# bitsauce/Carla-ppo

Measured on AMD Instinct MI355X. Metric: VAE+PPO train frames/sec on 160×80×3 synthetic obs at 1/2/4/8 MI355X, higher is better.
Workload: dtype bf16; 1 GPU; ConvVAE SGD step (fwd+ELBO+bwd+TF-Adam), batch=512 per GPU, 160x80x3 frames, z_dim=64, rgb target (BASELINE configs[1]; global batch 512); global_batch=512, parallelism=single, frames_resident_in_hbm=2048, frame_table=uint8 camera bytes, k/255 in registers, noise=N(0,1) drawn inside the reparameterisation kernel (Philox4x32-10), launch=eager launches: one C call per step (mi_vae_train_step), storage=bf16 activations/weights, fp32 accumulate, fp32 master weights+Adam

## Files before the change

### carla-ppo_amd/csrc/conv_ops.hip

```cpp
#include <stdlib.h>
#include "gemm_core.hpp"
#include "tallk_tile.hpp"
#include "mi_internal.hpp"
#include "mi355_carla.h"

using namespace mi;

namespace {

inline int esz_of(int dtype) { return dtype == MI_BF16 ? 2 : 4; }
inline bool dtype_ok(int dtype) { return dtype == MI_F32 || dtype == MI_BF16 || dtype == MI_BF16X3; }

template <typename T, typename TIn, int AMODE, int BMODE, int VA, int AALIGN>
int launch_gemm_bn(hipStream_t st, const GemmParams& p, int M_for_grid, int gz) {
    const int gx = (M_for_grid + GEMM_BM - 1) / GEMM_BM;
    if (gx <= 0) return MI_OK;
    if (p.N <= 32) {
        dim3 g(gx, 1, gz);
        MI_LAUNCH((gemm_kernel<T, TIn, AMODE, BMODE, VA, AALIGN, 32>), g, dim3(GEMM_NT), 0, st, p);
    } else if (p.N <= 64) {
        dim3 g(gx, 1, gz);
        MI_LAUNCH((gemm_kernel<T, TIn, AMODE, BMODE, VA, AALIGN, 64>), g, dim3(GEMM_NT), 0, st, p);
    } else {
        dim3 g(gx, (p.N + 127) / 128, gz);
// ... 835 lines not shown
}
extern "C" int mi_small_reduce_flush(void* stream) {
    if (t_sr.njobs == 0) return MI_OK;
    if ((hipStream_t)stream != t_sr_stream) {
        const int rc = sr_launch_params(t_sr_stream, t_sr);
        return rc != MI_OK ? rc : mi_fail(MI_ERR_STATE, "mi_small_reduce_flush: the recorded jobs belong to another stream (issued there)");
    }
    return sr_launch_params(t_sr_stream, t_sr);
}
extern "C" int mi_small_reduce_deferring(void) { return t_sr_defer; }

bool mi_narrow_enabled() { return narrow_enabled(); }

void mi_get_trace(long long** buf, int* cap) { *buf = g_trace; *cap = g_trace_cap; }

static bool tallk_enabled() {
    static int on = -1;
    if (on < 0) { const char* e = getenv("MI355_TALLK"); on = (e && e[0] == '0') ? 0 : 1; }
    return on != 0;
}

extern "C" {

int mi_debug_set_trace(void* dev_ptr, int capacity_entries) { g_trace = (long long*)dev_ptr; g_trace_cap = dev_ptr ? capacity_entries : 0; return MI_OK; }

int mi_set_tuning(int key, int value) {
    int prev;
    if (key == 0) { prev = gemm2_enabled() ? 1 : 0; g_gemm2_on = value ? 1 : 0; }
    else if (key == 1) { prev = tapconv_minblocks(); g_tap_min = value < 0 ? -1 : value; }
    else if (key == 2) { prev = g_wgrad_skip; g_wgrad_skip = value; }
    else if (key == 5) { prev = g_tap_variant; g_tap_variant = value; }
    else if (key == 6) { prev = g_tap_direct; g_tap_direct = value ? 1 : 0; }
    else if (key == 8) { prev = 0; }
    else if (key == 4) { prev = narrow_enabled() ? 1 : 0; g_narrow_on = value ? 1 : 0; }
    else if (key == 3) { prev = tapwgrad_enabled() ? 1 : 0; g_tapwgrad_on = value ? 1 : 0; }
    else if (key == 7) { prev = g_tapwgrad_split; g_tapwgrad_split = value ? 1 : 0; }
    else if (key == 9) { prev = g_tapwgrad_blocks; g_tapwgrad_blocks = value < 16 ? 16 : value; }
    else if (key == 10) { prev = g_nw_waves; g_nw_waves = value; }
    else if (key == 12) { prev = g_tap_mask_prefetch; g_tap_mask_prefetch = value ? 1 : 0; }
    else if (key == 11) { prev = g_dense_wgrad_blocks; g_dense_wgrad_blocks = value < 1 ? 1 : value; }
    else if (key == 13) { prev = mi_rwconv_mode(value < 0 ? 0 : value); }
    else if (key == 14) { prev = g_tapwgrad_cw; g_tapwgrad_cw = value ? 1 : 0; }
    else if (key == 15) { prev = mi_rwconv_conv_mode(value < 0 ? 0 : value); }
    else if (key == 16) { prev = mi_rwconv_blocks(value < 0 ? 0 : value); }
    else if (key == 17) { prev = g_gemm2_tile; g_gemm2_tile = value; }
    else if (key == 18) { prev = g_slab_bf16; g_slab_bf16 = value ? 1 : 0; }
    else if (key == 19) { prev = g_nw_depth; g_nw_depth = value; }
    else if (key == 20) { prev = g_gemm2_stages; g_gemm2_stages = value; }
    else if (key == 21) { prev = g_x3_tapwgrad; g_x3_tapwgrad = value; }
    else if (key == 22) { prev = g_dwgs_on; g_dwgs_on = value ? 1 : 0; }
    else if (key == 24) { prev = g_tw_ldec; g_tw_ldec = value < 0 || value > 3 ? 0 : value; }
    else if (key == 25) { prev = g_dectail_dbg; g_dectail_dbg = value; }
    else if (key == 26) { prev = g_dectail_split5; g_dectail_split5 = value ? 1 : 0; }
    else if (key == 23) { prev = mi_enc12_debug(value); }
    else return mi_fail(MI_ERR_ARG, "mi_set_tuning: unknown key");
    return prev;
}

int mi_conv2d_nhwc_fwd(void* stream, int dtype, const void* x, const int* frame_idx, int x_is_f32,
                       int B, int IH, int IW, int Cin, const void* w, int w_transposed, const float* bias, int KH, int KW, int Cout,
                       int relu, void* out) {
    return mi_conv2d_nhwc_fwd_bits(stream, dtype, x, frame_idx, x_is_f32, B, IH, IW, Cin, w, w_transposed, bias, KH, KW, Cout, relu, out, nullptr, nullptr);
}

int mi_conv2d_nhwc_fwd_bits(void* stream, int dtype, const void* x, const int* frame_idx, int x_is_f32,
                            int B, int IH, int IW, int Cin, const void* w, int w_transposed, const float* bias, int KH, int KW, int Cout,
                            int relu, void* out, void* relu_bits, int* wrote_bits) {
    const void* const wfrag = mi_rwconv_take_wfrag();
    const int OH = (IH - KH) / 2 + 1, OW = (IW - KW) / 2 + 1;
    if (wrote_bits) *wrote_bits = 0;
    if (w_transposed) {
        const int r4 = try_narrow_conv((hipStream_t)stream, dtype, x, x_is_f32 == 2 ? 2 : ((x_is_f32 || dtype == MI_F32) ? 1 : (dtype == MI_BF16X3 ? 3 : 0)), frame_idx, w, B, IH, IW, Cin, KH, KW, Cout, bias, relu, nullptr, out,
                                       (dtype == MI_BF16 && relu && Cout == 32) ? relu_bits : nullptr);
        if (r4 > 0 && wrote_bits && relu_bits && dtype == MI_BF16 && relu && Cout == 32) *wrote_bits = 1;
        if (r4 != 0) return r4 > 0 ? MI_OK : r4;
    }
    if (x_is_f32 == 2) return mi_fail(MI_ERR_ARG, "mi_conv2d_nhwc_fwd: uint8 frames are only read by the narrow-layer kernel (bf16 mode, 1..3 channels -> 32, K-contiguous weights)");
    GemmParams p = {};
    p.a = x; p.a_frame_idx = frame_idx;
    fill_conv_geom(p, B, IH, IW, Cin, OH, OW, KH, KW, 2, needs_merge(Cin, dtype, x_is_f32));
    p.N = Cout; p.b = w; p.ldb = w_transposed ? p.K : Cout; p.b_vec = vec_ok(w, p.ldb, dtype);
    p.out = out; p.bias = bias; p.mask = nullptr; p.relu = relu; p.out_f32 = 0; p.ksplit_len = 0;
    if (w_transposed) return conv_form_gemm<B_NK>((hipStream_t)stream, dtype, x_is_f32, p, 1, wfrag);
    return conv_form_gemm<B_KN>((hipStream_t)stream, dtype, x_is_f32, p, 1);
}

int mi_conv2d_nhwc_dgrad(void* stream, int dtype, const void* dy, int B, int OH, int OW, int Cout,
                         const void* w, int KH, int KW, int Cin, int IH, int IW, const void* mask, void* dx) {
    return mi_conv2d_nhwc_dgrad_bits(stream, dtype, dy, B, OH, OW, Cout, w, KH, KW, Cin, IH, IW, mask, nullptr, dx);
}

int mi_conv2d_nhwc_dgrad_bits(void* stream, int dtype, const void* dy, int B, int OH, int OW, int Cout,
                              const void* w, int KH, int KW, int Cin, int IH, int IW, const void* mask, const void* mask_bits, void* dx) {
    if (mask_bits) {
        const int r5 = mi_try_rwconv_gather((hipStream_t)stream, dtype, dy, w, B, OH, OW, Cout, IH, IW, Cin, KH, KW, dx, nullptr, mask, 0, mask_bits, nullptr, nullptr);
        if (r5 != 0) return r5 > 0 ? MI_OK : r5;
    }
    GemmParams p = {};
    p.a = dy; p.b = w; p.ldb = 0; p.b_vec = 1;
    p.out = dx; p.bias = nullptr; p.mask = mask; p.relu = 0; p.out_f32 = 0;
    return deconv_form_gemm((hipStream_t)stream, dtype, p, B, OH, OW, Cout, IH, IW, Cin, KH, KW);
}

int mi_conv2d_nhwc_wgrad(void* stream, int dtype, const void* x, const int* frame_idx, int x_is_f32,
                         int B, int IH, int IW, int Cin, const void* dy, int KH, int KW, int Cout, float* dw) {
    return mi_conv2d_nhwc_wgrad_ws(stream, dtype, x, frame_idx, x_is_f32, B, IH, IW, Cin, dy, KH, KW, Cout, dw, nullptr, 0, nullptr);
// ... 327 lines not shown
```

### carla-ppo_amd/csrc/enc12.hip

```cpp
#include <stdlib.h>
#include "enc12_tile.hpp"
#include "mi_internal.hpp"
#include "mi355_carla.h"

using namespace mi;

static int g_enc12_dbg = 0;
int mi_enc12_debug(int mask) { const int prev = g_enc12_dbg; g_enc12_dbg = mask < 0 ? 0 : mask; return prev; }

static int enc12_grid(int u8) {
    static int resident[2];
    if (!resident[u8]) {
        int per_cu = 0, dev = 0, cus = 256;
        hipDeviceProp_t pr;
        const void* fn = u8 ? (const void*)enc12_fwd_kernel<unsigned char> : (const void*)enc12_fwd_kernel<float>;
        if (hipOccupancyMaxActiveBlocksPerMultiprocessor(&per_cu, fn, 256, 0) != hipSuccess || per_cu < 1) per_cu = 2;
        if (hipGetDevice(&dev) == hipSuccess && hipGetDeviceProperties(&pr, dev) == hipSuccess) cus = pr.multiProcessorCount;
        resident[u8] = per_cu * cus;
    }
    return resident[u8];
}

extern "C" int mi_conv2d_enc12_fwd(void* stream, int dtype, const void* frames, int frames_fmt, const int* frame_idx, int B, int FH, int FW, const void* w1_t, const float* b1,
                                   const void* w2_t, const float* b2, void* act1, void* relu_bits1, void* act2, int* launched) {
    const void* const w2f = mi_rwconv_take_wfrag();
    if (!launched || !frames || !w1_t || !b1 || !w2_t || !b2 || !act1 || !act2) return mi_fail(MI_ERR_ARG, "mi_conv2d_enc12_fwd: missing buffers");
    *launched = 0;
    static int on = -1;
    if (on < 0) { const char* e = getenv("MI355_ENC12"); on = (e && e[0] == '0') ? 0 : 1; }
    if (!on || !mi_narrow_enabled() || dtype != MI_BF16 || (frames_fmt != 1 && frames_fmt != 2) || B < 1 || FH != 80 || FW != 160) return MI_OK;
    if ((((uintptr_t)frames) & (frames_fmt == 2 ? 1 : 7)) || (((uintptr_t)w1_t) | ((uintptr_t)w2_t) | ((uintptr_t)b1) | ((uintptr_t)b2) | ((uintptr_t)act1) | ((uintptr_t)act2)) & 15) return MI_OK;
    if (relu_bits1 && (((uintptr_t)relu_bits1) & 3)) return MI_OK;
    if ((long long)B * 3 >= (1ll << 30)) return MI_OK;
    Enc12Params q = {};
    q.frames = frames; q.frame_idx = frame_idx; q.frame_stride = (long long)FH * FW * 3;
    q.w1 = (const bf16_t*)w1_t; q.b1 = b1; q.w2 = (const bf16_t*)w2_t; q.b2 = b2;
    q.act1 = (bf16_t*)act1; q.bits1 = (uint32_t*)relu_bits1; q.act2 = (bf16_t*)act2;
    q.w2f = (const bf16_t*)w2f;
    q.B = B; q.ntiles = 3 * B;
    int nblocks = enc12_grid(frames_fmt == 2 ? 1 : 0);
    if (nblocks > q.ntiles) nblocks = q.ntiles;
    static int ring = -1;
    if (ring < 0) { const char* e = getenv("MI355_ENC12_RING"); ring = (e && e[0] == '0') ? 0 : 1; }
    static int c2 = -1;
    if (c2 < 0) { const char* e = getenv("MI355_ENC12_C2"); c2 = (e && e[0] == '0') ? 0 : 1; }
    int use_ring = ring, use_c2 = c2;
    int dbg = g_enc12_dbg;
    if (dbg & 4096) { use_ring = (dbg >> 13) & 1; use_c2 = (dbg >> 14) & 1; dbg = 0; }
    if (dbg && frames_fmt == 2) {
        q.dbg = dbg;
        if (dbg & 2048) MI_LAUNCH((enc12_fwd_kernel<unsigned char, 1, 1, 1>), dim3(nblocks), dim3(256), 0, (hipStream_t)stream, q);
        else MI_LAUNCH((enc12_fwd_kernel<unsigned char, 1>), dim3(nblocks), dim3(256), 0, (hipStream_t)stream, q);
    } else if (use_ring && use_c2 && frames_fmt == 2) MI_LAUNCH((enc12_fwd_kernel<unsigned char, 0, 1, 1>), dim3(nblocks), dim3(256), 0, (hipStream_t)stream, q);
    else if (use_ring && frames_fmt == 2) MI_LAUNCH((enc12_fwd_kernel<unsigned char, 0, 1>), dim3(nblocks), dim3(256), 0, (hipStream_t)stream, q);
    else if (frames_fmt == 2) MI_LAUNCH(enc12_fwd_kernel<unsigned char>, dim3(nblocks), dim3(256), 0, (hipStream_t)stream, q);
    else MI_LAUNCH(enc12_fwd_kernel<float>, dim3(nblocks), dim3(256), 0, (hipStream_t)stream, q);
    const int rc = mi_check_launch("enc12_fwd_kernel");
    if (rc == MI_OK) *launched = 1;
    return rc;
}
```

### carla-ppo_amd/csrc/enc12_tile.hpp

```cpp
#pragma once
#include "wgrad_tile.hpp"

namespace mi {

typedef uint32_t e12_u32x4 __attribute__((ext_vector_type(4)));

constexpr int E12_PW = 40;
constexpr int E12_ROWS = 15;
constexpr int E12_PLANE = E12_ROWS * E12_PW * 64;
constexpr int E12_LDS = 2 * E12_PLANE;

struct Enc12Params {
    const void* frames; const int* frame_idx; long long frame_stride;
    const bf16_t* w1; const float* b1;
    const bf16_t* w2; const float* b2;
    const bf16_t* w2f;
    bf16_t* act1; uint32_t* bits1;
    bf16_t* act2;
    int B, ntiles;
    int dbg;
};

template <int IMM> __device__ __forceinline__ void e12_lds_read(u16x8& d, uint32_t addr) { asm volatile("ds_read_b128 %0, %1 offset:%2" : "=&v"(d) : "v"(addr), "n"(IMM)); }
template <int N> __device__ __forceinline__ void e12_lds_wait(u16x8& d) { asm volatile("s_waitcnt lgkmcnt(%1)" : "+v"(d) : "n"(N)); }
template <int F> __device__ __forceinline__ void e12_frag_read(u16x8& d, const uint32_t (&base)[2][2]) {
    constexpr int kh = F >> 3, kw = (F >> 1) & 3, ks = F & 1;
    e12_lds_read<(kw & 1) * E12_PLANE + kh * E12_PW * 64>(d, base[kw >> 1][ks]);
}
template <int F, int NF> struct E12Conv2Pipe {
    static __device__ __forceinline__ void run(u16x8 (&fb)[NF], const u16x8 (&wf2)[32], f32x16& acc, const uint32_t (&base)[2][2]) {
        constexpr int issued = F == 0 ? NF - 1 : (F - 2 + NF < 31 ? F - 2 + NF : 31);
        e12_lds_wait<issued - F>(fb[F % NF]);
        acc = __builtin_amdgcn_mfma_f32_32x32x16_bf16(__builtin_bit_cast(bf16x8, wf2[F]), __builtin_bit_cast(bf16x8, fb[F % NF]), acc, 0, 0, 0);
        if constexpr (F >= 1 && F - 1 + NF < 32) e12_frag_read<F - 1 + NF>(fb[(F - 1) % NF], base);
        if constexpr (F + 1 < 32) E12Conv2Pipe<F + 1, NF>::run(fb, wf2, acc, base);
    }
};
template <int F, int NF> struct E12Conv2Prologue {
    static __device__ __forceinline__ void run(u16x8 (&fb)[NF], const uint32_t (&base)[2][2]) {
        e12_frag_read<F>(fb[F], base);
        if constexpr (F + 1 < NF) E12Conv2Prologue<F + 1, NF>::run(fb, base);
    }
};

template <typename TS, int DBG = 0, int RING = 0, int C2 = 0>
__global__ __launch_bounds__(256) __attribute__((amdgpu_waves_per_eu(2, 2))) void enc12_fwd_kernel(const Enc12Params p) {
    const int dbg = DBG ? p.dbg : 0;
    constexpr int SSZ = (int)sizeof(TS), GSZ = 4 * SSZ, GDW = GSZ / 4;
    constexpr int FW = 160, A1H = 39, A1W = 79, A2H = 18, A2W = 38;
    __shared__ __attribute__((aligned(1024))) unsigned char lds[E12_LDS];
    const int tid = threadIdx.x, lane = tid & 63;
    const int wave = __builtin_amdgcn_readfirstlane(tid >> 6);
    const int lrow = lane & 31, lgrp = lane >> 5;

    const int nt = wave & 1, mh = wave >> 1;
    u16x8 wf1[3], wf2[32];
    {
        const __amdgpu_buffer_rsrc_t rsW1 = __builtin_amdgcn_make_buffer_rsrc((void*)p.w1, 0, 32 * 48 * 2, 0x00020000);
        const bool w2frag = p.w2f != nullptr;
        const __amdgpu_buffer_rsrc_t rsW2 = __builtin_amdgcn_make_buffer_rsrc((void*)(w2frag ? p.w2f : p.w2), 0, 64 * 512 * 2, 0x00020000);
#pragma unroll
        for (int s = 0; s < 3; ++s) wf1[s] = __builtin_bit_cast(u16x8, __builtin_amdgcn_raw_buffer_load_b128(rsW1, (lrow * 48 + s * 16 + lgrp * 8) * 2, 0, 0));
#pragma unroll
        for (int f = 0; f < 32; ++f)
            wf2[f] = __builtin_bit_cast(u16x8, __builtin_amdgcn_raw_buffer_load_b128(rsW2, w2frag ? ((nt * 32 + f) * 64 + lane) * 16 : ((nt * 32 + lrow) * 512 + f * 16 + lgrp * 8) * 2, 0, 0));
    }
    f32x16 acc1_0, acc2_0;
#pragma unroll
    for (int qd = 0; qd < 4; ++qd) {
        const f32x4 ba = *(const f32x4*)(p.b1 + 8 * qd + 4 * lgrp), bb = *(const f32x4*)(p.b2 + nt * 32 + 8 * qd + 4 * lgrp);
#pragma unroll
        for (int t = 0; t < 4; ++t) { acc1_0[4 * qd + t] = ba[t]; acc2_0[4 * qd + t] = bb[t]; }
    }
    const uint32_t rowb = (uint32_t)(FW * 3 * SSZ);
    uint32_t goff[6];
#pragma unroll
    for (int j = 0; j < 6; ++j) {
        const int qa = 4 * (j >> 1) + (j & 1), qb = qa + 2;
        goff[j] = lgrp ? (uint32_t)(qb / 3) * rowb + (uint32_t)((qb % 3) * GSZ) : (uint32_t)(qa / 3) * rowb + (uint32_t)((qa % 3) * GSZ);
    }
    struct Raw { uint32_t d[6][GDW]; };

    const int G = (int)gridDim.x;
    struct Band { int b, band, y0, npix, own_rows, ngrp; const unsigned char* fbase; };
    auto band_of = [&](int tile) -> Band {
        Band q;
        q.b = tile / 3; q.band = tile - 3 * q.b; q.y0 = 12 * q.band;
        const int nrows = q.band == 2 ? 15 : 14;
        q.npix = nrows * A1W; q.own_rows = q.band == 2 ? 15 : 12;
        q.ngrp = (q.npix + 31) >> 5;
        long long fr = q.b;
        if constexpr (RING && SSZ == 1) {
            if (p.frame_idx) {
                int v;
                asm volatile("s_load_dword %0, %1, 0x0\n\ts_waitcnt lgkmcnt(0)" : "=s"(v) : "s"(p.frame_idx + q.b));
                fr = v;
            }
        } else if (p.frame_idx) fr = p.frame_idx[q.b];
        q.fbase = (const unsigned char*)p.frames + fr * p.frame_stride * SSZ;
        return q;
    };
    auto request3 = [&](const unsigned char* fbase, int y0r, int npixr, int grp, Raw& r) {
        const int pq = min(grp * 32 + lrow, npixr - 1);
        const int row = pq / A1W, col = pq - row * A1W;
        const unsigned char* pix = fbase + (2 * (y0r + row) * FW + 2 * col) * 3 * SSZ;
        if constexpr (RING && SSZ == 1) {
#pragma unroll
            for (int j = 0; j < 6; ++j) {
                if (dbg & 16) { r.d[j][0] = 0x40404040u + (uint32_t)pq; continue; }
                asm volatile("global_load_dword %0, %1, off" : "=&v"(r.d[j][0]) : "v"(pix + goff[j]));
            }
            return;
        }
#pragma unroll
        for (int j = 0; j < 6; ++j) {
            if (dbg & 16) {
#pragma unroll
                for (int e = 0; e < GDW; ++e) r.d[j][e] = 0x40404040u + (uint32_t)pq;
                continue;
            }
            const PackU<uint32_t, GDW, 2> v = *(const PackU<uint32_t, GDW, 2>*)(pix + goff[j]);
#pragma unroll
            for (int e = 0; e < GDW; ++e) r.d[j][e] = v.v[e];
        }
    };
    auto request = [&](const Band& q, int grp, Raw& r) { request3(q.fbase, q.y0, q.npix, grp, r); };
    auto ring_wait = [&](Raw& r) {
        if constexpr (RING && SSZ == 1)
            asm volatile("s_waitcnt vmcnt(%6)" : "+v"(r.d[0][0]), "+v"(r.d[1][0]), "+v"(r.d[2][0]), "+v"(r.d[3][0]), "+v"(r.d[4][0]), "+v"(r.d[5][0]) : "n"(6 * ((SSZ == 1 ? 3 : 2) - 1)));
    };
    constexpr bool DEEP = SSZ == 1;
    constexpr int NB = DEEP ? 3 : 2;
    Raw r0, r1, ra, rb, rc;
    int tile = (int)blockIdx.x;
    if (tile >= p.ntiles) return;
    Band cb = band_of(tile);
    if constexpr (RING) {
        request(cb, wave, ra); request(cb, wave + 4, rb);
        if constexpr (NB == 3) request(cb, wave + 8, rc);
    } else {
        request(cb, min(wave, cb.ngrp - 1), r0);
        if constexpr (DEEP) request(cb, min(wave + 4, cb.ngrp - 1), r1);
    }
    for (; tile < p.ntiles; tile += G) {
        const int b = cb.b, band = cb.band, y0 = cb.y0, npix = cb.npix, own_rows = cb.own_rows, ngrp = cb.ngrp;

        if constexpr (RING) {
            const int nsteps = (ngrp - wave + 3) >> 2, nsp = (nsteps + NB - 1) / NB * NB;
            const bool more = tile + G < p.ntiles;
            const Band nb = more ? band_of(tile + G) : cb;
            auto step = [&](Raw& cur, int k) {
                const int grp = wave + 4 * k;
                ring_wait(cur);
                u16x8 xf[3];
    #pragma unroll
                for (int j = 0; j < 6; ++j) {
                    uint32_t* dst = (uint32_t*)&xf[j >> 1] + 2 * (j & 1);
                    float f[4];
                    if constexpr (SSZ == 1) {
    #pragma unroll
                        for (int e = 0; e < 4; ++e) f[e] = (float)((cur.d[j][0] >> (8 * e)) & 255u) * U8_RCP255;
                    } else {
    #pragma unroll
                        for (int e = 0; e < 4; ++e) f[e] = __builtin_bit_cast(float, cur.d[j][e < GDW ? e : 0]);
// ... 188 lines not shown
```

### carla-ppo_amd/csrc/enchead.hip

```cpp
#include <stdlib.h>
#include "enchead_tile.hpp"
#include "mi_internal.hpp"
#include "mi355_carla.h"

using namespace mi;

namespace mi {
__global__ __launch_bounds__(1024) void enchead_reduce_kernel(const float* __restrict__ slabs, int n, float* __restrict__ dw, float* __restrict__ db) {
    __shared__ float red[32][33];
    const int c = threadIdx.x & 31, r0 = threadIdx.x >> 5;
    const bool bias = blockIdx.x == 48;
    const int col = bias ? 64 * 32 + c : (int)blockIdx.x * 32 + c;
    float s = 0.f;
    for (int k0 = r0; k0 < n; k0 += 256) {
        float v[8];
#pragma unroll
        for (int u = 0; u < 8; ++u) { const int k = k0 + 32 * u; v[u] = k < n ? __builtin_nontemporal_load(&slabs[(long long)k * EH_SLAB + col]) : 0.f; }
#pragma unroll
        for (int u = 0; u < 8; ++u) s += v[u];
    }
    red[r0][c] = s;
    __syncthreads();
    if (threadIdx.x < 32) {
        float t = 0.f;
#pragma unroll
        for (int r = 0; r < 32; ++r) t += red[r][threadIdx.x];
        if (bias) db[threadIdx.x] += t; else dw[col] += t;
    }
}
}

static int enchead_grid(int u8) {
    static int resident[2];
    if (!resident[u8]) {
        int per_cu = 0, dev = 0, cus = 256;
        hipDeviceProp_t pr;
        const void* fn = u8 ? (const void*)enchead_bwd_kernel<unsigned char> : (const void*)enchead_bwd_kernel<float>;
        if (hipOccupancyMaxActiveBlocksPerMultiprocessor(&per_cu, fn, 256, 0) != hipSuccess || per_cu < 1) per_cu = 2;
        if (hipGetDevice(&dev) == hipSuccess && hipGetDeviceProperties(&pr, dev) == hipSuccess) cus = pr.multiProcessorCount;
        resident[u8] = per_cu * cus;
    }
    return resident[u8];
}

extern "C" int mi_conv2d_head_bwd_blocks(void) { const int a = enchead_grid(0), b = enchead_grid(1); return a > b ? a : b; }

extern "C" int mi_conv2d_head_bwd_fused(void* stream, int dtype, const void* frames, int frames_fmt, const int* frame_idx, int B, int FH, int FW,
                                        const void* dy2, const void* w2, const void* bits_act1, float* dw1, float* db1, void* scratch, long long scratch_bytes, int* n_blocks) {
    if (!n_blocks || !frames || !dy2 || !w2 || !dw1 || !db1) return mi_fail(MI_ERR_ARG, "mi_conv2d_head_bwd_fused: missing buffers");
    *n_blocks = 0;
    static int on = -1;
    if (on < 0) { const char* e = getenv("MI355_ENCHEAD"); on = (e && e[0] == '0') ? 0 : 1; }
    if (!on || !mi_narrow_enabled() || dtype != MI_BF16 || !bits_act1 || !scratch || B < 1) return MI_OK;
    if (frames_fmt != 1 && frames_fmt != 2) return MI_OK;
    if (FH < 10 || FW < 10) return MI_OK;
    const int IH = (FH - 4) / 2 + 1, IW = (FW - 4) / 2 + 1;
    if (IH < 4 || IW < 4) return MI_OK;
    const int OH = (IH - 4) / 2 + 1, OW = (IW - 4) / 2 + 1;
    const int ssz = frames_fmt == 2 ? 1 : 4;
    if ((((uintptr_t)frames) & (2 * ssz - 1)) || ((long long)FW * 3 * ssz) % (2 * ssz) != 0 || ((long long)FH * FW * 3 * ssz) % (2 * ssz) != 0) return MI_OK;
    if ((((uintptr_t)dy2) | ((uintptr_t)w2) | ((uintptr_t)scratch) | ((uintptr_t)dw1) | ((uintptr_t)db1)) & 15) return MI_OK;
    if ((long long)B * OH * OW * 128 >= 0x7fffff00ll || (long long)B * IH * IW * 8 >= 0x7fffff00ll) return MI_OK;
    EncHeadParams q = {};
    q.dy = (const bf16_t*)dy2; q.dy_bytes = (unsigned)((long long)B * OH * OW * 128); q.B = B; q.OH = OH; q.OW = OW;
    q.w = (const bf16_t*)w2; q.bits = (const uint32_t*)bits_act1; q.bits_bytes = (unsigned)((long long)B * IH * IW * 8);
    q.frames = frames; q.frame_idx = frame_idx; q.frame_stride = (long long)FH * FW * 3;
    q.IH = IH; q.IW = IW; q.FW = FW;
    const int tiles_y = (IH + EH_TY - 1) / EH_TY;
    q.tiles_x = (IW + EH_TX - 1) / EH_TX; q.tiles_per_frame = tiles_y * q.tiles_x;
    const long long ntiles = (long long)B * q.tiles_per_frame;
    if (ntiles >= (1ll << 30)) return MI_OK;
    q.ntiles = (int)ntiles; q.div_tpf = make_fastdiv(q.tiles_per_frame); q.div_tx = make_fastdiv(q.tiles_x);
    int nblocks = enchead_grid(frames_fmt == 2 ? 1 : 0);
    if (nblocks > q.ntiles) nblocks = q.ntiles;
    if (nblocks >= 16) nblocks &= ~7;
    if (scratch_bytes < (long long)nblocks * EH_SLAB * 4) return MI_OK;
    q.slabs = (float*)scratch;
    hipStream_t st = (hipStream_t)stream;
    if (frames_fmt == 2) MI_LAUNCH(enchead_bwd_kernel<unsigned char>, dim3(nblocks), dim3(256), 0, st, q);
    else MI_LAUNCH(enchead_bwd_kernel<float>, dim3(nblocks), dim3(256), 0, st, q);
    int rc = mi_check_launch("enchead_bwd_kernel");
    if (rc != MI_OK) return rc;
    if (mi_small_reduce_deferring()) {
        rc = mi_reduce_slabs(st, q.slabs, (long long)EH_SLAB, nblocks, 48ll * 32, dw1);
        if (rc == MI_OK) rc = mi_reduce_slabs(st, q.slabs + 64 * 32, (long long)EH_SLAB, nblocks, 32ll, db1);
    } else {
        MI_LAUNCH(enchead_reduce_kernel, dim3(49), dim3(1024), 0, st, (const float*)q.slabs, nblocks, dw1, db1);
        rc = mi_check_launch("enchead_reduce_kernel");
    }
    if (rc == MI_OK) *n_blocks = nblocks;
    return rc;
}
```

### carla-ppo_amd/csrc/enchead_tile.hpp

```cpp
#pragma once
#include "wgrad_tile.hpp"

namespace mi {

constexpr int EH_TY = 8, EH_TX = 16;
constexpr int EH_SR = EH_TY / 2 + 1, EH_SC = EH_TX / 2 + 1;
constexpr int EH_NS = EH_SR * EH_SC;
constexpr int EH_SP = 144;
constexpr int EH_DYS = (EH_NS * EH_SP + 255) & ~255;
constexpr int EH_GP = 80;
constexpr int EH_GT = 32 * EH_GP;
constexpr int EH_SLAB = 64 * 32 + 32;
constexpr int EH_PT = 32 * 128;

struct EncHeadParams {
    const bf16_t* dy; unsigned dy_bytes; int B, OH, OW;
    const bf16_t* w;
    const uint32_t* bits; unsigned bits_bytes;
    const void* frames; const int* frame_idx; long long frame_stride;
    int IH, IW, FW;
    float* slabs;
    int tiles_x, tiles_per_frame, ntiles;
    FastDiv div_tpf, div_tx;
};

template <typename TS>
__global__ __launch_bounds__(256) __attribute__((amdgpu_waves_per_eu(3, 4))) void enchead_bwd_kernel(const EncHeadParams p) {
    constexpr int SSZ = (int)sizeof(TS), GSZ = 4 * SSZ, GDW = GSZ / 4;
    __shared__ __attribute__((aligned(1024))) unsigned char lds[EH_DYS + 4 * EH_PT + 4 * EH_GT + 4 * 4096];
    unsigned char* const dys = lds;
    const int tid = threadIdx.x, lane = tid & 63;
    const int wave = __builtin_amdgcn_readfirstlane(tid >> 6);
    const int lrow = lane & 31, lgrp = lane >> 5;
    unsigned char* const ptw = lds + EH_DYS + wave * EH_PT;
    unsigned char* const gtw = lds + EH_DYS + 4 * EH_PT + wave * EH_GT;
    const int ph = wave >> 1, pw = wave & 1;
    const int li = lrow >> 3, lj = lrow & 7;
    typedef __attribute__((address_space(3))) s16x4* lds_v4;

    unsigned char* const wlw = lds + EH_DYS + 4 * EH_PT + 4 * EH_GT + wave * 4096;
    u16x8 wf[3][4];
    {
        const __amdgpu_buffer_rsrc_t rsW = __builtin_amdgcn_make_buffer_rsrc((void*)p.w, 0, 16 * 32 * 64 * 2, 0x00020000);
#pragma unroll
        for (int tap = 0; tap < 4; ++tap) {
            const int kh = ph + 2 * (tap >> 1), kw = pw + 2 * (tap & 1);
#pragma unroll
            for (int kk = 0; kk < 4; ++kk) {
                const u16x8 f = __builtin_bit_cast(u16x8, __builtin_amdgcn_raw_buffer_load_b128(rsW, (((kh * 4 + kw) * 32 + lrow) * 64 + kk * 16 + lgrp * 8) * 2, 0, 0));
                if (tap < 3) wf[tap][kk] = f; else *(u16x8*)(wlw + kk * 1024 + lane * 16) = f;
            }
        }
    }
    {
        const f32x4 one_then_zero = {__builtin_bit_cast(float, 0x00003F80u), 0.f, 0.f, 0.f};
        *(f32x4*)(ptw + lrow * 128 + (((6 + lgrp) ^ (lrow & 7)) << 4)) = lgrp ? f32x4{0.f, 0.f, 0.f, 0.f} : one_then_zero;
    }
    f32x16 accw[2];
#pragma unroll
    for (int mt = 0; mt < 2; ++mt)
#pragma unroll
        for (int r = 0; r < 16; ++r) accw[mt][r] = 0.f;

    const __amdgpu_buffer_rsrc_t rsD = __builtin_amdgcn_make_buffer_rsrc((void*)p.dy, 0, (int)p.dy_bytes, 0x00020000);
    const __amdgpu_buffer_rsrc_t rsB = __builtin_amdgcn_make_buffer_rsrc((void*)p.bits, 0, (int)p.bits_bytes, 0x00020000);
    constexpr int EH_OOB = 0x7ffffff0;

    auto role = [&](int i, int& spix, int& schk, int& srow, int& scl, bool& sin) {
        const int id = tid + 256 * i; sin = id < EH_NS * 8; spix = sin ? id >> 3 : 0; schk = id & 7;
        srow = (spix * 57) >> 9; scl = spix - srow * EH_SC;
    };
    struct Staged { f32x4 d[2]; };
    auto tile_origin = [&](int tile, int& b, int& y0, int& x0) {
        uint32_t bb, rem, ty, tx;
        p.div_tpf.divmod((uint32_t)tile, bb, rem);
        p.div_tx.divmod(rem, ty, tx);
        b = (int)bb; y0 = (int)ty * EH_TY; x0 = (int)tx * EH_TX;
    };
    auto request = [&](int tile, Staged& R) {
        int b, y0, x0;
        tile_origin(tile, b, y0, x0);
#pragma unroll
        for (int i = 0; i < 2; ++i) {
            int spix, schk, srow, scl; bool sin;
            role(i, spix, schk, srow, scl, sin);
            const int oy = (y0 >> 1) - 1 + srow, ox = (x0 >> 1) - 1 + scl;
            const bool in = sin && (unsigned)oy < (unsigned)p.OH && (unsigned)ox < (unsigned)p.OW;
            const int off = in ? (((b * p.OH + oy) * p.OW + ox) * 64 + schk * 8) * 2 : EH_OOB;
            R.d[i] = __builtin_bit_cast(f32x4, __builtin_amdgcn_raw_buffer_load_b128(rsD, off, 0, 0));
        }
    };
    auto commit = [&](const Staged& R) {
#pragma unroll
        for (int i = 0; i < 2; ++i) {
            int spix, schk, srow, scl; bool sin;
            role(i, spix, schk, srow, scl, sin);
            if (sin) *(f32x4*)(dys + spix * EH_SP + schk * 16) = R.d[i];
        }
    };
    const uint32_t rowb = (uint32_t)(p.FW * 3 * SSZ);
    auto goff = [&](int j) -> uint32_t {
        const int qa = 4 * (j >> 1) + (j & 1), qb = qa + 2;
        const uint32_t oa = (uint32_t)(qa / 3) * rowb + (uint32_t)((qa % 3) * GSZ), ob = (uint32_t)(qb / 3) * rowb + (uint32_t)((qb % 3) * GSZ);
        return lgrp ? ob : oa;
    };
    struct Raw { uint32_t d[6][GDW]; uint32_t mw; };
    auto frame_of = [&](int b) -> int {
        int fr = b;
        if (p.frame_idx) asm volatile("s_load_dword %0, %1, 0x0\n\ts_waitcnt lgkmcnt(0)" : "=s"(fr) : "s"(p.frame_idx + b) : "memory");
        return fr;
    };
    auto request_patch = [&](int tile, Raw& r) {
        int b, y0, x0;
        tile_origin(tile, b, y0, x0);
        const int y = y0 + ph + 2 * li, x = x0 + pw + 2 * lj;
        const int yc = min(y, p.IH - 1), xc = min(x, p.IW - 1);
        const unsigned char* pix = (const unsigned char*)p.frames + ((long long)frame_of(b) * p.frame_stride + (2ll * yc * p.FW + 2 * xc) * 3) * SSZ;
#pragma unroll
        for (int j = 0; j < 6; ++j) {
            const PackU<uint32_t, GDW, 2> v = *(const PackU<uint32_t, GDW, 2>*)(pix + goff(j));
#pragma unroll
            for (int e = 0; e < GDW; ++e) r.d[j][e] = v.v[e];
        }
        const bool in = y < p.IH && x < p.IW;
        r.mw = __builtin_amdgcn_raw_buffer_load_b32(rsB, in ? (((b * p.IH + y) * p.IW + x) * 2 + lgrp) * 4 : EH_OOB, 0, 0);
    };

    const int G = (int)gridDim.x;
    const int vb = (G & 7) == 0 ? ((int)blockIdx.x & 7) * (G >> 3) + ((int)blockIdx.x >> 3) : (int)blockIdx.x;
    Staged cur;
    int t_nxt = min(vb + G, p.ntiles - 1);
    request(min(vb, p.ntiles - 1), cur);
    const uint32_t dya = (uint32_t)((li * EH_SC + lj) * EH_SP + lgrp * 16);
    const int tg = lane >> 4, tc = lane & 15;
    const int trow = (tg >> 1) * 8 + (tc >> 2), tcol = (tg & 1) * 16 + (tc & 3) * 4;

    Raw raw;
    request_patch(min(vb, p.ntiles - 1), raw);
    for (int tile = vb; tile < p.ntiles; tile += G) {
        commit(cur);
#pragma unroll
        for (int s = 0; s < 3; ++s) {
            u16x8 xf;
#pragma unroll
            for (int gi = 0; gi < 2; ++gi) {
                const int j = 2 * s + gi;
                float f[4];
                if constexpr (SSZ == 1) {
#pragma unroll
                    for (int e = 0; e < 4; ++e) f[e] = (float)((raw.d[j][0] >> (8 * e)) & 255u) * U8_RCP255;
                } else {
#pragma unroll
                    for (int e = 0; e < 4; ++e) f[e] = __builtin_bit_cast(float, raw.d[j][e < GDW ? e : 0]);
                }
                const PackN<uint32_t, 2> h = __builtin_bit_cast(PackN<uint32_t, 2>, pack4<bf16_t>(f));
                uint32_t* dst = (uint32_t*)&xf + 2 * gi;
                dst[0] = h.v[0]; dst[1] = h.v[1];
            }
            *(u16x8*)(ptw + lrow * 128 + (((2 * s + lgrp) ^ (lrow & 7)) << 4)) = xf;
        }
        const uint32_t mw = raw.mw;
        request_patch(t_nxt, raw);
        asm volatile("s_waitcnt lgkmcnt(0)\n\ts_barrier" ::: "memory");
        request(t_nxt, cur);
        t_nxt = min(t_nxt + G, p.ntiles - 1);

        f32x16 acc;
#pragma unroll
        for (int r = 0; r < 16; ++r) acc[r] = 0.f;
#pragma unroll
        for (int tap = 0; tap < 4; ++tap)
#pragma unroll
            for (int kk = 0; kk < 4; ++kk) {
                const u16x8 bf = *(const u16x8*)(dys + dya + ((1 - (tap >> 1)) * EH_SC + (1 - (tap & 1))) * EH_SP + kk * 32);
                u16x8 wa;
                if (tap < 3) wa = wf[tap][kk]; else wa = *(const u16x8*)(wlw + kk * 1024 + lane * 16);
                acc = __builtin_amdgcn_mfma_f32_32x32x16_bf16(__builtin_bit_cast(bf16x8, wa), __builtin_bit_cast(bf16x8, bf), acc, 0, 0, 0);
            }
        {
            uint32_t R[4][2];
#pragma unroll
            for (int qd = 0; qd < 4; ++qd) {
                const float v[4] = {acc[4 * qd], acc[4 * qd + 1], acc[4 * qd + 2], acc[4 * qd + 3]};
                const PackN<uint32_t, 2> w2 = __builtin_bit_cast(PackN<uint32_t, 2>, pack4<bf16_t>(v));
                R[qd][0] = w2.v[0]; R[qd][1] = w2.v[1];
            }
#pragma unroll
            for (int d = 0; d < 2; ++d) {
                auto r0 = __builtin_amdgcn_permlane32_swap(R[0][d], R[2][d], false, false); R[0][d] = r0[0]; R[2][d] = r0[1];
                auto r1 = __builtin_amdgcn_permlane32_swap(R[1][d], R[3][d], false, false); R[1][d] = r1[0]; R[3][d] = r1[1];
            }
            uint32_t o[8] = {R[0][0], R[0][1], R[2][0], R[2][1], R[1][0], R[1][1], R[3][0], R[3][1]};
#pragma unroll
            for (int d = 0; d < 8; ++d) o[d] &= ((mw >> d) & 0x00010001u) * 0xffffu;
            *(PackN<uint32_t, 4>*)(gtw + lrow * EH_GP + lgrp * 32) = PackN<uint32_t, 4>{{o[0], o[1], o[2], o[3]}};
            *(PackN<uint32_t, 4>*)(gtw + lrow * EH_GP + lgrp * 32 + 16) = PackN<uint32_t, 4>{{o[4], o[5], o[6], o[7]}};
        }
        __builtin_amdgcn_wave_barrier();
#pragma unroll
        for (int ks = 0; ks < 2; ++ks) {
            u16x8 bfr;
            {
                const int q0 = ks * 16 + trow, q1 = q0 + 4;
                const s16x4 lo = __builtin_amdgcn_ds_read_tr16_b64_v4i16((lds_v4)(gtw + q0 * EH_GP + tcol * 2));
                const s16x4 hi = __builtin_amdgcn_ds_read_tr16_b64_v4i16((lds_v4)(gtw + q1 * EH_GP + tcol * 2));
#pragma unroll
                for (int e = 0; e < 4; ++e) { bfr[e] = (unsigned short)lo[e]; bfr[4 + e] = (unsigned short)hi[e]; }
            }
#pragma unroll
            for (int mt = 0; mt < 2; ++mt) {
                const int col = mt * 32 + tcol;
                const int r0 = ks * 16 + trow, r1 = r0 + 4;
                const s16x4 lo = __builtin_amdgcn_ds_read_tr16_b64_v4i16((lds_v4)(ptw + r0 * 128 + (((col >> 3) ^ (r0 & 7)) << 4) + (col & 7) * 2));
                const s16x4 hi = __builtin_amdgcn_ds_read_tr16_b64_v4i16((lds_v4)(ptw + r1 * 128 + (((col >> 3) ^ (r1 & 7)) << 4) + (col & 7) * 2));
                u16x8 afr;
#pragma unroll
                for (int e = 0; e < 4; ++e) { afr[e] = (unsigned short)lo[e]; afr[4 + e] = (unsigned short)hi[e]; }
                accw[mt] = __builtin_amdgcn_mfma_f32_32x32x16_bf16(__builtin_bit_cast(bf16x8, afr), __builtin_bit_cast(bf16x8, bfr), accw[mt], 0, 0, 0);
// ... 31 lines not shown
```

### carla-ppo_amd/csrc/mi_internal.hpp

```cpp
#pragma once
#include <hip/hip_runtime.h>
#include <hip/hip_ext.h>

enum { MI_F32 = 0, MI_BF16 = 1, MI_BF16X3 = 2 };
enum { MI_OK = 0, MI_ERR_ARG = -1, MI_ERR_SHAPE = -2, MI_ERR_LAUNCH = -3, MI_ERR_STATE = -4 };

extern thread_local hipEvent_t mi_tl_stop_event;
#define MI_LAUNCH(kernel, grid, block, shmem, stream, ...) do { \
        if (mi_tl_stop_event) { const hipEvent_t ev__ = mi_tl_stop_event; mi_tl_stop_event = nullptr; \
            hipExtLaunchKernelGGL(kernel, grid, block, shmem, stream, nullptr, ev__, 0, __VA_ARGS__); } \
        else hipLaunchKernelGGL(kernel, grid, block, shmem, stream, __VA_ARGS__); } while (0)

const void* mi_rwconv_take_wfrag();
int mi_enc12_debug(int mask);
int mi_fail(int code, const char* msg);
int mi_check_launch(const char* what);

extern "C" int mi_tapwgrad_defer(int on);
extern "C" int mi_tapwgrad_flush(void* stream);
extern "C" int mi_tapwgrad_defer_pause(int pause);
extern "C" int mi_tapwgrad_slab_bf16(int on);

int mi_try_rwconv_gather(hipStream_t st, int dtype, const void* a, const void* w, int B, int IH, int IW, int C, int OH, int OW, int N,
                         int KH, int KW, void* out, const float* bias, const void* mask, int relu, const void* mask_bits, void* bits_out, const void* wfrag);
int mi_try_rwconv_conv(hipStream_t st, int dtype, const void* a, const void* w, int B, int IH, int IW, int C, int OH, int OW, int N,
                       int KH, int KW, int ldb, void* out, const float* bias, const void* mask, int relu, const void* wfrag);
int mi_rwconv_conv_mode(int set);
int mi_rwconv_blocks(int set);
int mi_rwconv_mode(int set);
void mi_get_trace(long long** buf, int* cap);

int mi_reduce_slabs(hipStream_t st, const float* slabs, long long stride, int nslab, long long n, float* out, int overwrite = 0);
extern "C" int mi_small_reduce_defer(int on);
extern "C" int mi_small_reduce_flush(void* stream);
extern "C" int mi_small_reduce_bind(void* stream);
extern "C" int mi_small_reduce_deferring(void);
bool mi_narrow_enabled();
```

Measured before the change: 644,900 frames/s.

## Stage camera-byte frame bands in LDS for encoder head backward and enc12 loads

Adds a BAND mode, on by default via MI355_ENC_BAND, in two kernels. In the enc12 forward ring loader, each thread issues six dword loads from a scalar frame base using immediate offsets, replacing the per-load 64-bit pointer arithmetic. In the encoder-head backward kernel, each tile's frame window is loaded cooperatively with coalesced dwords, converted to bf16 once into an extra LDS region, and the im2col patches are then built from LDS instead of six strided global loads per thread. This cuts redundant global traffic and address math, at the cost of more LDS per block (possibly lower occupancy) and extra LDS reads.

After: 645,600 frames/s (median of 6 runs). No clear change (+0.1%).

```diff
diff --git a/carla-ppo_amd/csrc/conv_ops.hip b/carla-ppo_amd/csrc/conv_ops.hip
--- a/carla-ppo_amd/csrc/conv_ops.hip
+++ b/carla-ppo_amd/csrc/conv_ops.hip
@@ -911,6 +911,7 @@
     else if (key == 24) { prev = g_tw_ldec; g_tw_ldec = value < 0 || value > 3 ? 0 : value; }
     else if (key == 25) { prev = g_dectail_dbg; g_dectail_dbg = value; }
     else if (key == 26) { prev = g_dectail_split5; g_dectail_split5 = value ? 1 : 0; }
+    else if (key == 27) { prev = mi_enc_band(value ? 1 : 0); }
     else if (key == 23) { prev = mi_enc12_debug(value); }
     else return mi_fail(MI_ERR_ARG, "mi_set_tuning: unknown key");
     return prev;
diff --git a/carla-ppo_amd/csrc/enc12.hip b/carla-ppo_amd/csrc/enc12.hip
--- a/carla-ppo_amd/csrc/enc12.hip
+++ b/carla-ppo_amd/csrc/enc12.hip
@@ -44,14 +44,16 @@
     if (ring < 0) { const char* e = getenv("MI355_ENC12_RING"); ring = (e && e[0] == '0') ? 0 : 1; }
     static int c2 = -1;
     if (c2 < 0) { const char* e = getenv("MI355_ENC12_C2"); c2 = (e && e[0] == '0') ? 0 : 1; }
-    int use_ring = ring, use_c2 = c2;
+    int use_ring = ring ? (mi_enc_band(-1) ? 2 : 1) : 0, use_c2 = c2;
     int dbg = g_enc12_dbg;
-    if (dbg & 4096) { use_ring = (dbg >> 13) & 1; use_c2 = (dbg >> 14) & 1; dbg = 0; }
+    if (dbg & 4096) { use_ring = ((dbg >> 13) & 1) ? (mi_enc_band(-1) ? 2 : 1) : 0; use_c2 = (dbg >> 14) & 1; dbg = 0; }
     if (dbg && frames_fmt == 2) {
         q.dbg = dbg;
         if (dbg & 2048) MI_LAUNCH((enc12_fwd_kernel<unsigned char, 1, 1, 1>), dim3(nblocks), dim3(256), 0, (hipStream_t)stream, q);
         else MI_LAUNCH((enc12_fwd_kernel<unsigned char, 1>), dim3(nblocks), dim3(256), 0, (hipStream_t)stream, q);
-    } else if (use_ring && use_c2 && frames_fmt == 2) MI_LAUNCH((enc12_fwd_kernel<unsigned char, 0, 1, 1>), dim3(nblocks), dim3(256), 0, (hipStream_t)stream, q);
+    } else if (use_ring == 2 && use_c2 && frames_fmt == 2) MI_LAUNCH((enc12_fwd_kernel<unsigned char, 0, 2, 1>), dim3(nblocks), dim3(256), 0, (hipStream_t)stream, q);
+    else if (use_ring == 2 && frames_fmt == 2) MI_LAUNCH((enc12_fwd_kernel<unsigned char, 0, 2>), dim3(nblocks), dim3(256), 0, (hipStream_t)stream, q);
+    else if (use_ring && use_c2 && frames_fmt == 2) MI_LAUNCH((enc12_fwd_kernel<unsigned char, 0, 1, 1>), dim3(nblocks), dim3(256), 0, (hipStream_t)stream, q);
     else if (use_ring && frames_fmt == 2) MI_LAUNCH((enc12_fwd_kernel<unsigned char, 0, 1>), dim3(nblocks), dim3(256), 0, (hipStream_t)stream, q);
     else if (frames_fmt == 2) MI_LAUNCH(enc12_fwd_kernel<unsigned char>, dim3(nblocks), dim3(256), 0, (hipStream_t)stream, q);
     else MI_LAUNCH(enc12_fwd_kernel<float>, dim3(nblocks), dim3(256), 0, (hipStream_t)stream, q);
diff --git a/carla-ppo_amd/csrc/enc12_tile.hpp b/carla-ppo_amd/csrc/enc12_tile.hpp
--- a/carla-ppo_amd/csrc/enc12_tile.hpp
+++ b/carla-ppo_amd/csrc/enc12_tile.hpp
@@ -21,6 +21,9 @@
     int dbg;
 };
 
+template <int IMM> __device__ __forceinline__ void e12_gload(uint32_t& d, uint32_t voff, const unsigned char* base) {
+    asm volatile("global_load_dword %0, %1, %2 offset:%3" : "=&v"(d) : "v"(voff), "s"(base), "n"(IMM));
+}
 template <int IMM> __device__ __forceinline__ void e12_lds_read(u16x8& d, uint32_t addr) { asm volatile("ds_read_b128 %0, %1 offset:%2" : "=&v"(d) : "v"(addr), "n"(IMM)); }
 template <int N> __device__ __forceinline__ void e12_lds_wait(u16x8& d) { asm volatile("s_waitcnt lgkmcnt(%1)" : "+v"(d) : "n"(N)); }
 template <int F> __device__ __forceinline__ void e12_frag_read(u16x8& d, const uint32_t (&base)[2][2]) {
@@ -105,11 +108,28 @@
         const int row = pq / A1W, col = pq - row * A1W;
         const unsigned char* pix = fbase + (2 * (y0r + row) * FW + 2 * col) * 3 * SSZ;
         if constexpr (RING && SSZ == 1) {
-#pragma unroll
-            for (int j = 0; j < 6; ++j) {
-                if (dbg & 16) { r.d[j][0] = 0x40404040u + (uint32_t)pq; continue; }
-                asm volatile("global_load_dword %0, %1, off" : "=&v"(r.d[j][0]) : "v"(pix + goff[j]));
-            }
+            if constexpr (RING == 1) {
+#pragma unroll
+                for (int j = 0; j < 6; ++j) {
+                    if (dbg & 16) { r.d[j][0] = 0x40404040u + (uint32_t)pq; continue; }
+                    asm volatile("global_load_dword %0, %1, off" : "=&v"(r.d[j][0]) : "v"(pix + goff[j]));
+                }
+                return;
+            }
+            if (dbg & 16) {
+#pragma unroll
+                for (int j = 0; j < 6; ++j) r.d[j][0] = 0x40404040u + (uint32_t)pq;
+                return;
+            }
+            constexpr int RB = FW * 3;
+            const uint32_t po = 6u * ((uint32_t)pq + __umul24((uint32_t)row, (uint32_t)(FW - A1W)) + __umul24((uint32_t)y0r, (uint32_t)FW));
+            const uint32_t va = po + (lgrp ? 8u : 0u), vb = po + (lgrp ? (uint32_t)(RB - 4) : 0u);
+            e12_gload<0>(r.d[0][0], va, fbase);
+            e12_gload<4>(r.d[1][0], vb, fbase);
+            e12_gload<RB + 4>(r.d[2][0], vb, fbase);
+            e12_gload<RB + 8>(r.d[3][0], vb, fbase);
+            e12_gload<2 * RB + 8>(r.d[4][0], vb, fbase);
+            e12_gload<3 * RB>(r.d[5][0], va, fbase);
             return;
         }
 #pragma unroll
diff --git a/carla-ppo_amd/csrc/enchead.hip b/carla-ppo_amd/csrc/enchead.hip
--- a/carla-ppo_amd/csrc/enchead.hip
+++ b/carla-ppo_amd/csrc/enchead.hip
@@ -30,20 +30,30 @@
 }
 }
 
-static int enchead_grid(int u8) {
-    static int resident[2];
-    if (!resident[u8]) {
+static int g_enc_band = -1;
+int mi_enc_band(int on) {
+    if (g_enc_band < 0) { const char* e = getenv("MI355_ENC_BAND"); g_enc_band = (e && e[0] == '0') ? 0 : 1; }
+    const int prev = g_enc_band;
+    if (on >= 0) g_enc_band = on;
+    return prev;
+}
+
+static const void* enchead_fn(int form) {
+    return form == 2 ? (const void*)enchead_bwd_kernel<unsigned char, 1> : form == 1 ? (const void*)enchead_bwd_kernel<unsigned char> : (const void*)enchead_bwd_kernel<float>;
+}
+static int enchead_grid(int form) {
+    static int resident[3];
+    if (!resident[form]) {
         int per_cu = 0, dev = 0, cus = 256;
         hipDeviceProp_t pr;
-        const void* fn = u8 ? (const void*)enchead_bwd_kernel<unsigned char> : (const void*)enchead_bwd_kernel<float>;
-        if (hipOccupancyMaxActiveBlocksPerMultiprocessor(&per_cu, fn, 256, 0) != hipSuccess || per_cu < 1) per_cu = 2;
+        if (hipOccupancyMaxActiveBlocksPerMultiprocessor(&per_cu, enchead_fn(form), 256, 0) != hipSuccess || per_cu < 1) per_cu = 2;
         if (hipGetDevice(&dev) == hipSuccess && hipGetDeviceProperties(&pr, dev) == hipSuccess) cus = pr.multiProcessorCount;
-        resident[u8] = per_cu * cus;
+        resident[form] = per_cu * cus;
     }
-    return resident[u8];
+    return resident[form];
 }
 
-extern "C" int mi_conv2d_head_bwd_blocks(void) { const int a = enchead_grid(0), b = enchead_grid(1); return a > b ? a : b; }
+extern "C" int mi_conv2d_head_bwd_blocks(void) { int m = 0; for (int f = 0; f < 3; ++f) { const int n = enchead_grid(f); if (n > m) m = n; } return m; }
 
 extern "C" int mi_conv2d_head_bwd_fused(void* stream, int dtype, const void* frames, int frames_fmt, const int* frame_idx, int B, int FH, int FW,
                                         const void* dy2, const void* w2, const void* bits_act1, float* dw1, float* db1, void* scratch, long long scratch_bytes, int* n_blocks) {
@@ -65,19 +75,21 @@
     q.dy = (const bf16_t*)dy2; q.dy_bytes = (unsigned)((long long)B * OH * OW * 128); q.B = B; q.OH = OH; q.OW = OW;
     q.w = (const bf16_t*)w2; q.bits = (const uint32_t*)bits_act1; q.bits_bytes = (unsigned)((long long)B * IH * IW * 8);
     q.frames = frames; q.frame_idx = frame_idx; q.frame_stride = (long long)FH * FW * 3;
-    q.IH = IH; q.IW = IW; q.FW = FW;
+    q.IH = IH; q.IW = IW; q.FH = FH; q.FW = FW;
     const int tiles_y = (IH + EH_TY - 1) / EH_TY;
     q.tiles_x = (IW + EH_TX - 1) / EH_TX; q.tiles_per_frame = tiles_y * q.tiles_x;
     const long long ntiles = (long long)B * q.tiles_per_frame;
     if (ntiles >= (1ll << 30)) return MI_OK;
     q.ntiles = (int)ntiles; q.div_tpf = make_fastdiv(q.tiles_per_frame); q.div_tx = make_fastdiv(q.tiles_x);
-    int nblocks = enchead_grid(frames_fmt == 2 ? 1 : 0);
+    const int form = frames_fmt != 2 ? 0 : (mi_enc_band(-1) && !(((uintptr_t)frames) & 3) && (FW * 3) % 4 == 0) ? 2 : 1;
+    int nblocks = enchead_grid(form);
     if (nblocks > q.ntiles) nblocks = q.ntiles;
     if (nblocks >= 16) nblocks &= ~7;
     if (scratch_bytes < (long long)nblocks * EH_SLAB * 4) return MI_OK;
     q.slabs = (float*)scratch;
     hipStream_t st = (hipStream_t)stream;
-    if (frames_fmt == 2) MI_LAUNCH(enchead_bwd_kernel<unsigned char>, dim3(nblocks), dim3(256), 0, st, q);
+    if (form == 2) MI_LAUNCH((enchead_bwd_kernel<unsigned char, 1>), dim3(nblocks), dim3(256), 0, st, q);
+    else if (form == 1) MI_LAUNCH(enchead_bwd_kernel<unsigned char>, dim3(nblocks), dim3(256), 0, st, q);
     else MI_LAUNCH(enchead_bwd_kernel<float>, dim3(nblocks), dim3(256), 0, st, q);
     int rc = mi_check_launch("enchead_bwd_kernel");
     if (rc != MI_OK) return rc;
diff --git a/carla-ppo_amd/csrc/enchead_tile.hpp b/carla-ppo_amd/csrc/enchead_tile.hpp
--- a/carla-ppo_amd/csrc/enchead_tile.hpp
+++ b/carla-ppo_amd/csrc/enchead_tile.hpp
@@ -12,22 +12,27 @@
 constexpr int EH_GT = 32 * EH_GP;
 constexpr int EH_SLAB = 64 * 32 + 32;
 constexpr int EH_PT = 32 * 128;
+constexpr int EH_FR = 2 * EH_TY + 2;
+constexpr int EH_FD = ((2 * EH_TX + 2) * 3 + 3) / 4;
+constexpr int EH_FP = EH_FD * 8;
+constexpr int EH_FWIN = EH_FR * EH_FP;
 
 struct EncHeadParams {
     const bf16_t* dy; unsigned dy_bytes; int B, OH, OW;
     const bf16_t* w;
     const uint32_t* bits; unsigned bits_bytes;
     const void* frames; const int* frame_idx; long long frame_stride;
-    int IH, IW, FW;
+    int IH, IW, FH, FW;
     float* slabs;
     int tiles_x, tiles_per_frame, ntiles;
     FastDiv div_tpf, div_tx;
 };
 
-template <typename TS>
+template <typename TS, int BAND = 0>
 __global__ __launch_bounds__(256) __attribute__((amdgpu_waves_per_eu(3, 4))) void enchead_bwd_kernel(const EncHeadParams p) {
     constexpr int SSZ = (int)sizeof(TS), GSZ = 4 * SSZ, GDW = GSZ / 4;
-    __shared__ __attribute__((aligned(1024))) unsigned char lds[EH_DYS + 4 * EH_PT + 4 * EH_GT + 4 * 4096];
+    static_assert(!BAND || SSZ == 1, "the frame stager takes camera bytes");
+    __shared__ __attribute__((aligned(1024))) unsigned char lds[EH_DYS + 4 * EH_PT + 4 * EH_GT + 4 * 4096 + (BAND ? EH_FWIN : 0)];
     unsigned char* const dys = lds;
     const int tid = threadIdx.x, lane = tid & 63;
     const int wave = __builtin_amdgcn_readfirstlane(tid >> 6);
@@ -104,23 +109,36 @@
         const uint32_t oa = (uint32_t)(qa / 3) * rowb + (uint32_t)((qa % 3) * GSZ), ob = (uint32_t)(qb / 3) * rowb + (uint32_t)((qb % 3) * GSZ);
         return lgrp ? ob : oa;
     };
-    struct Raw { uint32_t d[6][GDW]; uint32_t mw; };
+    struct Raw { uint32_t d[BAND ? 2 : 6][BAND ? 1 : GDW]; uint32_t mw; };
     auto frame_of = [&](int b) -> int {
         int fr = b;
         if (p.frame_idx) asm volatile("s_load_dword %0, %1, 0x0\n\ts_waitcnt lgkmcnt(0)" : "=s"(fr) : "s"(p.frame_idx + b) : "memory");
         return fr;
     };
+    auto win_item = [&](int i, int& wr, int& wd) { const int it = min(tid + 256 * i, EH_FR * EH_FD - 1); wr = it / EH_FD; wd = it - wr * EH_FD; };
+    unsigned char* const win = lds + EH_DYS + 4 * EH_PT + 4 * EH_GT + 4 * 4096;
     auto request_patch = [&](int tile, Raw& r) {
         int b, y0, x0;
         tile_origin(tile, b, y0, x0);
         const int y = y0 + ph + 2 * li, x = x0 + pw + 2 * lj;
-        const int yc = min(y, p.IH - 1), xc = min(x, p.IW - 1);
-        const unsigned char* pix = (const unsigned char*)p.frames + ((long long)frame_of(b) * p.frame_stride + (2ll * yc * p.FW + 2 * xc) * 3) * SSZ;
-#pragma unroll
-        for (int j = 0; j < 6; ++j) {
-            const PackU<uint32_t, GDW, 2> v = *(const PackU<uint32_t, GDW, 2>*)(pix + goff(j));
-#pragma unroll
-            for (int e = 0; e < GDW; ++e) r.d[j][e] = v.v[e];
+        if constexpr (BAND) {
+            const unsigned char* fb = (const unsigned char*)p.frames + (long long)frame_of(b) * p.frame_stride;
+#pragma unroll
+            for (int i = 0; i < 2; ++i) {
+                int wr, wd;
+                win_item(i, wr, wd);
+                const int fy = min(2 * y0 + wr, p.FH - 1), fc = min(6 * x0 + 4 * wd, (int)rowb - 4);
+                r.d[i][0] = *(const uint32_t*)(fb + (uint32_t)fy * rowb + (uint32_t)fc);
+            }
+        } else {
+            const int yc = min(y, p.IH - 1), xc = min(x, p.IW - 1);
+            const unsigned char* pix = (const unsigned char*)p.frames + ((long long)frame_of(b) * p.frame_stride + (2ll * yc * p.FW + 2 * xc) * 3) * SSZ;
+#pragma unroll
+            for (int j = 0; j < 6; ++j) {
+                const PackU<uint32_t, GDW, 2> v = *(const PackU<uint32_t, GDW, 2>*)(pix + goff(j));
+#pragma unroll
+                for (int e = 0; e < GDW; ++e) r.d[j][e] = v.v[e];
+            }
         }
         const bool in = y < p.IH && x < p.IW;
         r.mw = __builtin_amdgcn_raw_buffer_load_b32(rsB, in ? (((b * p.IH + y) * p.IW + x) * 2 + lgrp) * 4 : EH_OOB, 0, 0);
@@ -139,6 +157,17 @@
     request_patch(min(vb, p.ntiles - 1), raw);
     for (int tile = vb; tile < p.ntiles; tile += G) {
         commit(cur);
+        if constexpr (BAND) {
+#pragma unroll
+            for (int i = 0; i < 2; ++i) {
+                int wr, wd;
+                win_item(i, wr, wd);
+                float f[4];
+#pragma unroll
+                for (int e = 0; e < 4; ++e) f[e] = (float)((raw.d[i][0] >> (8 * e)) & 255u) * U8_RCP255;
+                *(PackN<bf16_t, 4>*)(win + wr * EH_FP + wd * 8) = pack4<bf16_t>(f);
+            }
+        } else
 #pragma unroll
         for (int s = 0; s < 3; ++s) {
             u16x8 xf;
@@ -164,6 +193,21 @@
         asm volatile("s_waitcnt lgkmcnt(0)\n\ts_barrier" ::: "memory");
         request(t_nxt, cur);
         t_nxt = min(t_nxt + G, p.ntiles - 1);
+        if constexpr (BAND) {
+            const unsigned char* wl = win + (2 * ph + 4 * li) * EH_FP + (pw + 2 * lj) * 12;
+#pragma unroll
+            for (int s = 0; s < 3; ++s) {
+                u16x8 xf;
+#pragma unroll
+                for (int gi = 0; gi < 2; ++gi) {
+                    const int qa = 4 * s + gi, qb = qa + 2;
+                    const uint32_t* src = (const uint32_t*)(wl + (lgrp ? (qb / 3) * EH_FP + (qb % 3) * 8 : (qa / 3) * EH_FP + (qa % 3) * 8));
+                    uint32_t* dst = (uint32_t*)&xf + 2 * gi;
+                    dst[0] = src[0]; dst[1] = src[1];
+                }
+                *(u16x8*)(ptw + lrow * 128 + (((2 * s + lgrp) ^ (lrow & 7)) << 4)) = xf;
+            }
+        }
 
         f32x16 acc;
 #pragma unroll
diff --git a/carla-ppo_amd/csrc/mi_internal.hpp b/carla-ppo_amd/csrc/mi_internal.hpp
--- a/carla-ppo_amd/csrc/mi_internal.hpp
+++ b/carla-ppo_amd/csrc/mi_internal.hpp
@@ -13,6 +13,7 @@
 
 const void* mi_rwconv_take_wfrag();
 int mi_enc12_debug(int mask);
+int mi_enc_band(int on);
 int mi_fail(int code, const char* msg);
 int mi_check_launch(const char* what);
 
```
